# NazirNayal8/RbA

Hardware: AMD Instinct MI355X
Metric: images/sec @1024x2048 Swin-B-1dl (RbA inference hot path) (higher is better)
Workload: dtype f32 (f16x3 split-MFMA GEMMs, fp32 accumulate)

## Files before the change

### rba_amd/csrc/build.py

```python
import os
import subprocess
import sys
from concurrent.futures import ThreadPoolExecutor

HERE = os.path.dirname(os.path.abspath(__file__))
SOURCES = ["rba_reduce.hip", "rba_reduce_bwd.hip", "resample.hip", "ms_deform_attn.hip", "ms_deform_attn_bwd.hip", "masked_xattn.hip", "mask_logits.hip", "mask_logits_bwd.hip", "point_loss.hip", "outlier_tail.hip", "dense_hybrid_loss.hip", "pebal_loss.hip", "tta_merge.hip", "resize_u8.hip", "confusion.hip", "train_view.hip",
           "swin_window_attn.hip", "swin_attn_block.hip", "group_norm.hip", "layer_norm.hip", "skinny_linear.hip", "split_linear.hip", "split_linear_dma.hip", "split_linear_gnf.hip", "gaussian_blur.hip", "open_panoptic.hip", "dense_hybrid.hip", "patch_embed.hip", "token_linear.hip", "decoder_small.hip"]
HEADERS = ["common.h", "knobs.h", "bilinear_ac.h", "rba_reduce_kernels.h", "split_linear_dma.h", "split_linear_h3.h", "split_linear_h3q.h", "mlp_fused_h3.h", "swin_window_attn_h3.h", "swin_attn_block.h",
           os.path.join("..", "..", "include", "rba_hip.h")]
TUNE_SOURCES = [os.path.join("tune", "rba_reduce_tune.hip"), os.path.join("tune", "split_linear_tune.hip"), os.path.join("tune", "split_linear_ws.hip"), os.path.join("tune", "mlp_fused_h1.hip"), os.path.join("tune", "k5_timing.hip"), os.path.join("tune", "k5_wpe_ab.hip"), os.path.join("tune", "k5_wpe_plain.hip"), os.path.join("tune", "k5_persist.hip"), os.path.join("tune", "k7_timing.hip")] + [os.path.join("tune", f"gnf_form{f}_dbg{d}.hip") for f in (0, 1) for d in (0, 1)] + [os.path.join("tune", "gnf_form0_dbg1_unpacked.hip"), os.path.join("tune", "gnf_form1_dbg0_unpacked.hip")]
TUNE_LIB = os.path.join(HERE, "tune", "librba_tune.so")
LIB = os.path.join(HERE, "librba_hip.so")
KNOBS_LIB = os.path.join(HERE, "librba_hip_knobs.so")
KNOBS = ["-DRBA_TUNE_KNOBS"]
OBJ = os.path.join(HERE, "build")
HIPCC = os.environ.get("HIPCC", "/opt/rocm/bin/hipcc")
FLAGS = ["--offload-arch=gfx950", "-O3", "-std=c++17", "-fPIC", "-ffp-contract=fast", "-Wno-unused-result"]
NO_PACKED_FP32 = ["-Xclang", "-target-feature", "-Xclang", "-packed-fp32-ops"]
MFMA_SOURCES = ({"split_linear.hip", "split_linear_dma.hip", "mask_logits.hip", "mask_logits_bwd.hip", "masked_xattn.hip", "skinny_linear.hip"}
                if os.environ.get("RBA_NO_PACKED_FP32") == "1" else set())
UNPACKED_ALWAYS = {"split_linear_gnf.hip", "ms_deform_attn_bwd.hip", "point_loss.hip", "outlier_tail.hip", "dense_hybrid_loss.hip"}
UNPACKED_SOURCES = MFMA_SOURCES | UNPACKED_ALWAYS


def _run(cmd):
    r = subprocess.run(cmd, cwd=HERE, stderr=subprocess.PIPE, text=True)
    err = "\n".join(ln for ln in r.stderr.splitlines() if "not a recognized feature for this target" not in ln)
    if err.strip():
        print(err, file=sys.stderr, flush=True)
    if r.returncode:
        raise subprocess.CalledProcessError(r.returncode, cmd)


def _stale(target, deps) -> bool:
    if not os.path.exists(target):
        return True
    t = os.path.getmtime(target)
    return any(os.path.getmtime(d) > t for d in deps)


def stale() -> bool:
    return _stale(LIB, [os.path.join(HERE, f) for f in SOURCES + HEADERS])


def build(force: bool = False, verbose: bool = True, knobs: bool = False) -> str:
    lib = KNOBS_LIB if knobs else LIB
    if not force and not _stale(lib, [os.path.join(HERE, f) for f in SOURCES + HEADERS]):
        return lib
    obj_dir = os.path.join(OBJ, "knobs") if knobs else OBJ
    os.makedirs(obj_dir, exist_ok=True)
    hdrs = [os.path.join(HERE, h) for h in HEADERS]

    def compile_one(src):
        s, o = os.path.join(HERE, src), os.path.join(obj_dir, src.replace(".hip", ".o"))
        if force or _stale(o, [s] + hdrs):
            cmd = [HIPCC] + FLAGS + (KNOBS if knobs else []) + (NO_PACKED_FP32 if src in UNPACKED_SOURCES else []) + ["-c", s, "-o", o]
            if verbose:
                print(" ".join(cmd), flush=True)
            _run(cmd)
        return o

    with ThreadPoolExecutor(max_workers=min(8, os.cpu_count() or 1)) as ex:
        objs = list(ex.map(compile_one, SOURCES))
    _link_and_gate(objs, lib, verbose)
    return lib


def _link_and_gate(objs, lib, verbose):
    tmp = lib + ".unscanned"
    cmd = [HIPCC, "--offload-arch=gfx950", "-shared", "-fPIC"] + objs + ["-o", tmp]
    if verbose:
        print(" ".join(cmd), flush=True)
    subprocess.run(cmd, check=True, cwd=HERE)
    try:
        from . import isa_hazards
    except ImportError:
        sys.path.insert(0, HERE)
        import isa_hazards
    try:
        r = isa_hazards.gate(tmp)
    except Exception:
        os.remove(tmp)
        raise
    if verbose:
        print(f"isa_hazards: {os.path.basename(lib)}: {r['code_objects']} code objects clean (rules D, T, P)", flush=True)
    os.replace(tmp, lib)


def build_knobs(force: bool = False, verbose: bool = True) -> str:
    return build(force=force, verbose=verbose, knobs=True)


def build_tune(force: bool = False, verbose: bool = True) -> str:
    deps = [os.path.join(HERE, f) for f in TUNE_SOURCES + HEADERS + [os.path.join("tune", "split_linear_experiments.h"), os.path.join("tune", "rba_reduce_experiments.h")]]
    if not force and not _stale(TUNE_LIB, deps):
        return TUNE_LIB
    os.makedirs(OBJ, exist_ok=True)
    objs = []
    for src in TUNE_SOURCES:
        o = os.path.join(OBJ, "tune_" + os.path.basename(src).replace(".hip", ".o"))
        cmd = [HIPCC] + FLAGS + KNOBS + (NO_PACKED_FP32 if (MFMA_SOURCES and "split_linear" in src) or src.endswith("split_linear_ws.hip") or src.endswith("_unpacked.hip") or (src.endswith("mlp_fused_h1.hip") and os.environ.get("RBA_MLP1_UNPACKED") == "1") else []) + ["-c", os.path.join(HERE, src), "-o", o]
        if verbose:
            print(" ".join(cmd), flush=True)
        _run(cmd)
        objs.append(o)
    cmd = [HIPCC, "--offload-arch=gfx950", "-shared", "-fPIC"] + objs + ["-o", TUNE_LIB]
    if verbose:
        print(" ".join(cmd), flush=True)
    subprocess.run(cmd, check=True, cwd=HERE)
    return TUNE_LIB


if __name__ == "__main__":
    print(build(force="--force" in sys.argv))
    if "--knobs" in sys.argv:
        print(build_knobs(force="--force" in sys.argv))
    if "--tune" in sys.argv:
        print(build_tune(force="--force" in sys.argv))
```

### rba_amd/csrc/resample.hip

```cpp
#include "common.h"
#include "../../include/rba_hip.h"

namespace {

constexpr int CCHUNK = 4;

template <bool ADD, bool VEC4>
__global__ __launch_bounds__(256) void resample_kernel(const float* __restrict__ in, const float* __restrict__ add,
                                                       float* __restrict__ out, int C, int h, int w, int H, int W,
                                                       float sh, float sw, int wq) {
  const int xg = blockIdx.x * blockDim.x + threadIdx.x;
  const int y = blockIdx.y;
  if (xg >= wq) return;
  const int x0 = xg * 4;
  const BilinearTap ty = bilinear_tap(y, sh, h);
  BilinearTap tx[4];
#pragma unroll
  for (int r = 0; r < 4; ++r) tx[r] = bilinear_tap(x0 + r < W ? x0 + r : W - 1, sw, w);
  const int c0 = blockIdx.z * CCHUNK;
  auto one = [&](int c) {
    const float* r0 = in + ((int64_t)c * h + ty.i0) * w;
    const float* r1 = in + ((int64_t)c * h + ty.i1) * w;
    float v[4];
#pragma unroll
    for (int r = 0; r < 4; ++r) {
      const float top = tx[r].l0 * r0[tx[r].i0] + tx[r].l1 * r0[tx[r].i1];
      const float bot = tx[r].l0 * r1[tx[r].i0] + tx[r].l1 * r1[tx[r].i1];
      v[r] = ty.l0 * top + ty.l1 * bot;
    }
    const int64_t o = ((int64_t)c * H + y) * W + x0;
    if (VEC4) {
      f32x4 t = {v[0], v[1], v[2], v[3]};
      if (ADD) {
        t += *reinterpret_cast<const f32x4*>(add + o);
        *reinterpret_cast<f32x4*>(out + o) = t;
      } else {
        __builtin_nontemporal_store(t, reinterpret_cast<f32x4*>(out + o));
      }
    } else {
#pragma unroll
      for (int r = 0; r < 4; ++r)
        if (x0 + r < W) out[o + r] = ADD ? v[r] + add[o + r] : v[r];
    }
  };
  if (c0 + CCHUNK <= C) {
#pragma unroll
    for (int i = 0; i < CCHUNK; ++i) one(c0 + i);
  } else {
    for (int c = c0; c < C; ++c) one(c);
  }
}

struct GnFold {
  const float* mr;
  const float* gamma;
  const float* beta;
  int cpg;
  int relu;
};
__device__ __forceinline__ void gn_fold_coeff(const GnFold& g, int j, f32x4& a, f32x4& b) {
  const int grp = (j << 2) / g.cpg;
  const float mean = g.mr[2 * grp], rstd = g.mr[2 * grp + 1];
  const f32x4 ga = reinterpret_cast<const f32x4*>(g.gamma)[j], be = reinterpret_cast<const f32x4*>(g.beta)[j];
#pragma unroll
  for (int k = 0; k < 4; ++k) {
    a[k] = ga[k] * rstd;
    b[k] = be[k] - mean * a[k];
  }
}
__device__ __forceinline__ f32x4 gn_fold_apply(f32x4 v, const f32x4 a, const f32x4 b, int relu) {
#pragma unroll
  for (int k = 0; k < 4; ++k) {
    v[k] = fmaf(v[k], a[k], b[k]);
    v[k] = rba_clamp_below(v[k], rba_relu_floor(relu));
  }
  return v;
}

template <bool ADD, bool SOUT = false, bool GN = false>
__global__ __launch_bounds__(256) void resample_nhwc_kernel(const float* __restrict__ in, const float* __restrict__ add,
                                                            float* __restrict__ out, int C4, int h, int w, int H, int W, float sh,
                                                            float sw, int64_t row0 = 0, GnFold gin = GnFold{nullptr, nullptr, nullptr, 4, 0},
                                                            GnFold gadd = GnFold{nullptr, nullptr, nullptr, 4, 0}) {
  int64_t idx = (int64_t)blockIdx.x * 256 + threadIdx.x;
  int j;
  int64_t pix;
  if (SOUT) {
    const int64_t wv = idx >> 6;
    const int ln = (int)(idx & 63), nblk = C4 >> 3;
    j = (int)(wv % nblk) * 8 + (ln & 7);
    pix = (wv / nblk) * 8 + (ln >> 3);
    if (pix >= (int64_t)H * W) return;
    idx = pix * C4 + j;
  } else {
    const int64_t total = (int64_t)H * W * C4;
    if (idx >= total) return;
    j = (int)(idx % C4);
    pix = idx / C4;
  }
  const int x = (int)(pix % W), y = (int)(pix / W);
  const BilinearTap ty = bilinear_tap(y, sh, h), tx = bilinear_tap(x, sw, w);
  const f32x4* ip = reinterpret_cast<const f32x4*>(in) + j;
  f32x4 v00 = ip[((int64_t)ty.i0 * w + tx.i0) * C4], v01 = ip[((int64_t)ty.i0 * w + tx.i1) * C4];
  f32x4 v10 = ip[((int64_t)ty.i1 * w + tx.i0) * C4], v11 = ip[((int64_t)ty.i1 * w + tx.i1) * C4];
  if (GN && gin.mr) {
    f32x4 a, b;
    gn_fold_coeff(gin, j, a, b);
    v00 = gn_fold_apply(v00, a, b, gin.relu);
    v01 = gn_fold_apply(v01, a, b, gin.relu);
    v10 = gn_fold_apply(v10, a, b, gin.relu);
    v11 = gn_fold_apply(v11, a, b, gin.relu);
  }
  f32x4 r;
#pragma unroll
  for (int k = 0; k < 4; ++k) {
    const float top = tx.l0 * v00[k] + tx.l1 * v01[k];
    const float bot = tx.l0 * v10[k] + tx.l1 * v11[k];
    r[k] = ty.l0 * top + ty.l1 * bot;
  }
  if (ADD) {
    f32x4 av = reinterpret_cast<const f32x4*>(add)[idx];
    if (GN && gadd.mr) {
      f32x4 a, b;
      gn_fold_coeff(gadd, j, a, b);
      av = gn_fold_apply(av, a, b, gadd.relu);
    }
    r += av;
  }
  if (SOUT) {
    uint32_t hh[2], ll[2];
    rba_split_f16x2(r.x, r.y, hh[0], ll[0]);
    rba_split_f16x2(r.z, r.w, hh[1], ll[1]);
    const bool odd = j & 1;
    const uint32_t s0 = odd ? hh[0] : ll[0], s1 = odd ? hh[1] : ll[1];
    const uint32_t r0 = __builtin_amdgcn_mov_dpp(s0, 0xB1, 0xf, 0xf, true), r1 = __builtin_amdgcn_mov_dpp(s1, 0xB1, 0xf, 0xf, true);
    const rba_u32x4 piece = odd ? (rba_u32x4){r0, r1, ll[0], ll[1]} : (rba_u32x4){hh[0], hh[1], r0, r1};
    const int64_t row = row0 + pix;
    const int k8 = j >> 1;
    const int64_t off = ((row >> 5) * (int64_t)(C4 >> 3) + (k8 >> 2)) * 4096 + ((k8 & 1) * 2 + (odd ? 1 : 0)) * 1024 +
                        (((k8 >> 1) & 1) * 32 + (int)(row & 31)) * 16;
    *reinterpret_cast<rba_u32x4*>(reinterpret_cast<char*>(out) + off) = piece;
  } else {
    reinterpret_cast<f32x4*>(out)[idx] = r;
  }
}

}

extern "C" int rba_resample_bilinear_f32(const float* in, const float* add, float* out, int C, int h, int w, int H, int W,
                                         void* stream) {
  RBA_CHECK_ARG(C >= 0 && h >= 1 && w >= 1 && H >= 0 && W >= 0 && H <= 65535);
  if (C == 0 || H == 0 || W == 0) return 0;
  RBA_CHECK_ARG(in && out);
  const int cz = (C + CCHUNK - 1) / CCHUNK;
  RBA_CHECK_ARG(cz <= 65535);
  rba_begin();
  hipStream_t st = (hipStream_t)stream;
  const int wq = (W + 3) / 4;
  const int threads = wq >= 256 ? 256 : (wq >= 128 ? 128 : 64);
  dim3 grid((wq + threads - 1) / threads, H, cz);
  const float sh = (float)h / (float)H, sw = (float)w / (float)W;
  const bool vec4 = (W % 4 == 0) && ((((uintptr_t)out | (uintptr_t)add) & 15) == 0);
#define RBA_L(A, V) hipLaunchKernelGGL((resample_kernel<A, V>), grid, dim3(threads), 0, st, in, add, out, C, h, w, H, W, sh, sw, wq)
  if (add && vec4) RBA_L(true, true);
  else if (add) RBA_L(true, false);
  else if (vec4) RBA_L(false, true);
  else RBA_L(false, false);
#undef RBA_L
  return rba_launch_status();
}

extern "C" int rba_resample_bilinear_nhwc_f32(const float* in, const float* add, float* out, int C, int h, int w, int H, int W,
                                              void* stream) {
  RBA_CHECK_ARG(C >= 0 && (C & 3) == 0 && h >= 1 && w >= 1 && H >= 0 && W >= 0);
  if (C == 0 || H == 0 || W == 0) return 0;
  RBA_CHECK_ARG(in && out && ((((uintptr_t)in | (uintptr_t)out | (uintptr_t)add) & 15) == 0));
  const int64_t total = (int64_t)H * W * (C >> 2);
  RBA_CHECK_ARG((total + 255) / 256 <= 0x7fffffff);
  rba_begin();
  const float sh = (float)h / (float)H, sw = (float)w / (float)W;
  const dim3 grid((unsigned)((total + 255) / 256));
  if (add)
    hipLaunchKernelGGL(resample_nhwc_kernel<true>, grid, dim3(256), 0, (hipStream_t)stream, in, add, out, C >> 2, h, w, H, W, sh, sw);
  else
    hipLaunchKernelGGL(resample_nhwc_kernel<false>, grid, dim3(256), 0, (hipStream_t)stream, in, add, out, C >> 2, h, w, H, W, sh, sw);
  return rba_launch_status();
}

extern "C" int rba_resample_bilinear_nhwc_split_out_f32(const float* in, const float* add, void* out_frag, int C, int h, int w, int H, int W,
                                                        int64_t row0, void* stream) {
  RBA_CHECK_ARG(C >= 32 && (C % 32) == 0 && h >= 1 && w >= 1 && H >= 0 && W >= 0 && row0 >= 0);
  if (H == 0 || W == 0) return 0;
  RBA_CHECK_ARG(in && out_frag && (((uintptr_t)in | (uintptr_t)add | (uintptr_t)out_frag) & 15) == 0);
  const int64_t total = (((int64_t)H * W + 7) / 8) * 8 * (C >> 2);
  RBA_CHECK_ARG((total + 255) / 256 <= 0x7fffffffLL);
  rba_begin();
  const float sh = (float)h / (float)H, sw = (float)w / (float)W;
  const dim3 grid((unsigned)((total + 255) / 256));
  float* o = reinterpret_cast<float*>(out_frag);
  if (add)
    hipLaunchKernelGGL((resample_nhwc_kernel<true, true>), grid, dim3(256), 0, (hipStream_t)stream, in, add, o, C >> 2, h, w, H, W, sh, sw, row0);
  else
    hipLaunchKernelGGL((resample_nhwc_kernel<false, true>), grid, dim3(256), 0, (hipStream_t)stream, in, add, o, C >> 2, h, w, H, W, sh, sw, row0);
  return rba_launch_status();
}

extern "C" int rba_resample_bilinear_nhwc_gn_f32(const float* in, const float* in_mr, const float* in_gamma, const float* in_beta, int in_relu,
                                                 const float* add, const float* add_mr, const float* add_gamma, const float* add_beta, void* out,
                                                 int split_out, int C, int G, int h, int w, int H, int W, int64_t row0, void* stream) {
  RBA_CHECK_ARG(C >= 4 && (C % 4) == 0 && G >= 1 && (C % G) == 0 && ((C / G) % 4) == 0 && h >= 1 && w >= 1 && H >= 0 && W >= 0 && row0 >= 0);
  RBA_CHECK_ARG(!split_out || (C % 32) == 0);
  if (H == 0 || W == 0) return 0;
  RBA_CHECK_ARG(in && add && out && (!in_mr || (in_gamma && in_beta)) && (!add_mr || (add_gamma && add_beta)));
  RBA_CHECK_ARG((((uintptr_t)in | (uintptr_t)add | (uintptr_t)out | (uintptr_t)in_gamma | (uintptr_t)in_beta | (uintptr_t)add_gamma | (uintptr_t)add_beta) & 15) == 0);
  const int64_t total = split_out ? (((int64_t)H * W + 7) / 8) * 8 * (C >> 2) : (int64_t)H * W * (C >> 2);
  RBA_CHECK_ARG((total + 255) / 256 <= 0x7fffffffLL);
  rba_begin();
  const float sh = (float)h / (float)H, sw = (float)w / (float)W;
  const dim3 grid((unsigned)((total + 255) / 256));
  const GnFold gi{in_mr, in_gamma, in_beta, C / G, in_relu}, ga{add_mr, add_gamma, add_beta, C / G, 0};
  float* o = reinterpret_cast<float*>(out);
  if (split_out)
    hipLaunchKernelGGL((resample_nhwc_kernel<true, true, true>), grid, dim3(256), 0, (hipStream_t)stream, in, add, o, C >> 2, h, w, H, W, sh, sw, row0, gi, ga);
  else
    hipLaunchKernelGGL((resample_nhwc_kernel<true, false, true>), grid, dim3(256), 0, (hipStream_t)stream, in, add, o, C >> 2, h, w, H, W, sh, sw, row0, gi, ga);
  return rba_launch_status();
}
```

Before: 151.0.

## Compute multiple output rows per thread in GN-fused NHWC bilinear resample

Replaces the per-pixel GN-fused NHWC resample with a kernel where each thread handles R consecutive output rows (2 or 4) for one column and channel quad. For 2x upsampling with aligned taps, it loads R/2+1 source rows once and reuses the horizontally interpolated values across output rows, cutting redundant input loads and GN-fold arithmetic. The GN coefficient loads are hoisted and made branch-free, and a heuristic or knob picks R. A frozen copy of the old kernel is added to the tune library for comparison. The cost is more register pressure and a duplicated clamped-row path.

```diff
diff --git a/rba_amd/csrc/build.py b/rba_amd/csrc/build.py
--- a/rba_amd/csrc/build.py
+++ b/rba_amd/csrc/build.py
@@ -8,7 +8,7 @@
            "swin_window_attn.hip", "swin_attn_block.hip", "group_norm.hip", "layer_norm.hip", "skinny_linear.hip", "split_linear.hip", "split_linear_dma.hip", "split_linear_gnf.hip", "gaussian_blur.hip", "open_panoptic.hip", "dense_hybrid.hip", "patch_embed.hip", "token_linear.hip", "decoder_small.hip"]
 HEADERS = ["common.h", "knobs.h", "bilinear_ac.h", "rba_reduce_kernels.h", "split_linear_dma.h", "split_linear_h3.h", "split_linear_h3q.h", "mlp_fused_h3.h", "swin_window_attn_h3.h", "swin_attn_block.h",
            os.path.join("..", "..", "include", "rba_hip.h")]
-TUNE_SOURCES = [os.path.join("tune", "rba_reduce_tune.hip"), os.path.join("tune", "split_linear_tune.hip"), os.path.join("tune", "split_linear_ws.hip"), os.path.join("tune", "mlp_fused_h1.hip"), os.path.join("tune", "k5_timing.hip"), os.path.join("tune", "k5_wpe_ab.hip"), os.path.join("tune", "k5_wpe_plain.hip"), os.path.join("tune", "k5_persist.hip"), os.path.join("tune", "k7_timing.hip")] + [os.path.join("tune", f"gnf_form{f}_dbg{d}.hip") for f in (0, 1) for d in (0, 1)] + [os.path.join("tune", "gnf_form0_dbg1_unpacked.hip"), os.path.join("tune", "gnf_form1_dbg0_unpacked.hip")]
+TUNE_SOURCES = [os.path.join("tune", "rba_reduce_tune.hip"), os.path.join("tune", "split_linear_tune.hip"), os.path.join("tune", "split_linear_ws.hip"), os.path.join("tune", "mlp_fused_h1.hip"), os.path.join("tune", "k5_timing.hip"), os.path.join("tune", "k5_wpe_ab.hip"), os.path.join("tune", "k5_wpe_plain.hip"), os.path.join("tune", "k5_persist.hip"), os.path.join("tune", "k7_timing.hip"), os.path.join("tune", "fpn_path_frozen.hip")] + [os.path.join("tune", f"gnf_form{f}_dbg{d}.hip") for f in (0, 1) for d in (0, 1)] + [os.path.join("tune", "gnf_form0_dbg1_unpacked.hip"), os.path.join("tune", "gnf_form1_dbg0_unpacked.hip")]
 TUNE_LIB = os.path.join(HERE, "tune", "librba_tune.so")
 LIB = os.path.join(HERE, "librba_hip.so")
 KNOBS_LIB = os.path.join(HERE, "librba_hip_knobs.so")
diff --git a/rba_amd/csrc/resample.hip b/rba_amd/csrc/resample.hip
--- a/rba_amd/csrc/resample.hip
+++ b/rba_amd/csrc/resample.hip
@@ -1,5 +1,7 @@
 #include "common.h"
 #include "../../include/rba_hip.h"
+
+RBA_KNOB(rba_resample_rows, 0);
 
 namespace {
 
@@ -51,37 +53,24 @@
   }
 }
 
-struct GnFold {
-  const float* mr;
-  const float* gamma;
-  const float* beta;
-  int cpg;
-  int relu;
-};
-__device__ __forceinline__ void gn_fold_coeff(const GnFold& g, int j, f32x4& a, f32x4& b) {
-  const int grp = (j << 2) / g.cpg;
-  const float mean = g.mr[2 * grp], rstd = g.mr[2 * grp + 1];
-  const f32x4 ga = reinterpret_cast<const f32x4*>(g.gamma)[j], be = reinterpret_cast<const f32x4*>(g.beta)[j];
-#pragma unroll
-  for (int k = 0; k < 4; ++k) {
-    a[k] = ga[k] * rstd;
-    b[k] = be[k] - mean * a[k];
-  }
-}
-__device__ __forceinline__ f32x4 gn_fold_apply(f32x4 v, const f32x4 a, const f32x4 b, int relu) {
-#pragma unroll
-  for (int k = 0; k < 4; ++k) {
-    v[k] = fmaf(v[k], a[k], b[k]);
-    v[k] = rba_clamp_below(v[k], rba_relu_floor(relu));
-  }
-  return v;
-}
-
-template <bool ADD, bool SOUT = false, bool GN = false>
+__device__ __forceinline__ void resample_store_split(const f32x4 r, float* out, int64_t row, int j, int C4) {
+  uint32_t hh[2], ll[2];
+  rba_split_f16x2(r.x, r.y, hh[0], ll[0]);
+  rba_split_f16x2(r.z, r.w, hh[1], ll[1]);
+  const bool odd = j & 1;
+  const uint32_t s0 = odd ? hh[0] : ll[0], s1 = odd ? hh[1] : ll[1];
+  const uint32_t r0 = __builtin_amdgcn_mov_dpp(s0, 0xB1, 0xf, 0xf, true), r1 = __builtin_amdgcn_mov_dpp(s1, 0xB1, 0xf, 0xf, true);
+  const rba_u32x4 piece = odd ? (rba_u32x4){r0, r1, ll[0], ll[1]} : (rba_u32x4){hh[0], hh[1], r0, r1};
+  const int k8 = j >> 1;
+  const int64_t off = ((row >> 5) * (int64_t)(C4 >> 3) + (k8 >> 2)) * 4096 + ((k8 & 1) * 2 + (odd ? 1 : 0)) * 1024 +
+                      (((k8 >> 1) & 1) * 32 + (int)(row & 31)) * 16;
+  *reinterpret_cast<rba_u32x4*>(reinterpret_cast<char*>(out) + off) = piece;
+}
+
+template <bool ADD, bool SOUT = false>
 __global__ __launch_bounds__(256) void resample_nhwc_kernel(const float* __restrict__ in, const float* __restrict__ add,
                                                             float* __restrict__ out, int C4, int h, int w, int H, int W, float sh,
-                                                            float sw, int64_t row0 = 0, GnFold gin = GnFold{nullptr, nullptr, nullptr, 4, 0},
-                                                            GnFold gadd = GnFold{nullptr, nullptr, nullptr, 4, 0}) {
+                                                            float sw, int64_t row0 = 0) {
   int64_t idx = (int64_t)blockIdx.x * 256 + threadIdx.x;
   int j;
   int64_t pix;
@@ -103,14 +92,6 @@
   const f32x4* ip = reinterpret_cast<const f32x4*>(in) + j;
   f32x4 v00 = ip[((int64_t)ty.i0 * w + tx.i0) * C4], v01 = ip[((int64_t)ty.i0 * w + tx.i1) * C4];
   f32x4 v10 = ip[((int64_t)ty.i1 * w + tx.i0) * C4], v11 = ip[((int64_t)ty.i1 * w + tx.i1) * C4];
-  if (GN && gin.mr) {
-    f32x4 a, b;
-    gn_fold_coeff(gin, j, a, b);
-    v00 = gn_fold_apply(v00, a, b, gin.relu);
-    v01 = gn_fold_apply(v01, a, b, gin.relu);
-    v10 = gn_fold_apply(v10, a, b, gin.relu);
-    v11 = gn_fold_apply(v11, a, b, gin.relu);
-  }
   f32x4 r;
 #pragma unroll
   for (int k = 0; k < 4; ++k) {
@@ -118,31 +99,150 @@
     const float bot = tx.l0 * v10[k] + tx.l1 * v11[k];
     r[k] = ty.l0 * top + ty.l1 * bot;
   }
-  if (ADD) {
-    f32x4 av = reinterpret_cast<const f32x4*>(add)[idx];
-    if (GN && gadd.mr) {
-      f32x4 a, b;
-      gn_fold_coeff(gadd, j, a, b);
-      av = gn_fold_apply(av, a, b, gadd.relu);
-    }
-    r += av;
-  }
+  if (ADD) r += reinterpret_cast<const f32x4*>(add)[idx];
   if (SOUT) {
-    uint32_t hh[2], ll[2];
-    rba_split_f16x2(r.x, r.y, hh[0], ll[0]);
-    rba_split_f16x2(r.z, r.w, hh[1], ll[1]);
-    const bool odd = j & 1;
-    const uint32_t s0 = odd ? hh[0] : ll[0], s1 = odd ? hh[1] : ll[1];
-    const uint32_t r0 = __builtin_amdgcn_mov_dpp(s0, 0xB1, 0xf, 0xf, true), r1 = __builtin_amdgcn_mov_dpp(s1, 0xB1, 0xf, 0xf, true);
-    const rba_u32x4 piece = odd ? (rba_u32x4){r0, r1, ll[0], ll[1]} : (rba_u32x4){hh[0], hh[1], r0, r1};
-    const int64_t row = row0 + pix;
-    const int k8 = j >> 1;
-    const int64_t off = ((row >> 5) * (int64_t)(C4 >> 3) + (k8 >> 2)) * 4096 + ((k8 & 1) * 2 + (odd ? 1 : 0)) * 1024 +
-                        (((k8 >> 1) & 1) * 32 + (int)(row & 31)) * 16;
-    *reinterpret_cast<rba_u32x4*>(reinterpret_cast<char*>(out) + off) = piece;
+    resample_store_split(r, out, row0 + pix, j, C4);
   } else {
     reinterpret_cast<f32x4*>(out)[idx] = r;
   }
+}
+
+struct GnFold {
+  const float* mr;
+  const float* gamma;
+  const float* beta;
+  int cpg;
+  int relu;
+};
+struct GnRaw {
+  float mean, rstd;
+  f32x4 ga, be;
+};
+__device__ __forceinline__ GnRaw gn_fold_load(const GnFold& g, int j, const float* safe) {
+  const bool on = g.mr != nullptr;
+  const float* mr = on ? g.mr : safe;
+  const int grp = (j << 2) / g.cpg;
+  return GnRaw{mr[2 * grp], mr[2 * grp + 1], reinterpret_cast<const f32x4*>(on ? g.gamma : safe)[j], reinterpret_cast<const f32x4*>(on ? g.beta : safe)[j]};
+}
+__device__ __forceinline__ void gn_fold_coeff(const GnRaw& g, f32x4& a, f32x4& b) {
+#pragma unroll
+  for (int k = 0; k < 4; ++k) {
+    a[k] = g.ga[k] * g.rstd;
+    b[k] = fmaf(-g.mean, a[k], g.be[k]);
+  }
+}
+template <bool CLAMP>
+__device__ __forceinline__ f32x4 gn_fold_apply(f32x4 v, const f32x4 a, const f32x4 b, float floor = 0.f) {
+#pragma unroll
+  for (int k = 0; k < 4; ++k) {
+    v[k] = fmaf(v[k], a[k], b[k]);
+    if (CLAMP) v[k] = rba_clamp_below(v[k], floor);
+  }
+  return v;
+}
+
+__device__ __forceinline__ BilinearTap resample_tap(int dst, float scale, int in_size) {
+  float src = fmaf(scale, (float)dst + 0.5f, -0.5f);
+  src = src < 0.0f ? 0.0f : src;
+  int i0 = (int)src;
+  i0 = i0 < in_size - 1 ? i0 : in_size - 1;
+  BilinearTap t;
+  t.i0 = i0;
+  t.i1 = i0 < in_size - 1 ? i0 + 1 : i0;
+  t.l1 = src - (float)i0;
+  t.l0 = 1.0f - t.l1;
+  return t;
+}
+
+__device__ __forceinline__ f32x4 resample_lerp(float l0, const f32x4 a, float l1, const f32x4 b) {
+  return (f32x4){fmaf(l1, b.x, l0 * a.x), fmaf(l0, a.y, l1 * b.y), fmaf(l1, b.z, l0 * a.z), fmaf(l0, a.w, l1 * b.w)};
+}
+
+template <bool SOUT, int R>
+__global__ __launch_bounds__(256) void resample_nhwc_gn_kernel(const float* __restrict__ in, const float* __restrict__ add, float* __restrict__ out, int C4, int h,
+                                                               int w, int H, int W, float sh, float sw, int64_t row0, GnFold gin, GnFold gadd) {
+  constexpr int NS = R / 2 + 1;
+  int x, j;
+  if (SOUT) {
+    const unsigned wv = blockIdx.x * 4 + (threadIdx.x >> 6), nblk = (unsigned)C4 >> 3, xg = wv / nblk;
+    const int ln = threadIdx.x & 63;
+    j = (int)(wv - xg * nblk) * 8 + (ln & 7);
+    x = (int)xg * 8 + (ln >> 3);
+    if (x >= W) return;
+  } else {
+    const unsigned e = blockIdx.x * 256 + threadIdx.x;
+    if (e >= (unsigned)W * (unsigned)C4) return;
+    x = (int)(e / (unsigned)C4);
+    j = (int)(e - (unsigned)x * (unsigned)C4);
+  }
+  const int ya = R * (int)blockIdx.y - 1;
+  const BilinearTap tx = resample_tap(x, sw, w);
+  const f32x4* ip = reinterpret_cast<const f32x4*>(in) + j;
+  const f32x4* ap = reinterpret_cast<const f32x4*>(add) + j;
+  int pix[R];
+  BilinearTap ty[R];
+  f32x4 av[R];
+#pragma unroll
+  for (int r = 0; r < R; ++r) {
+    const int y = ya + r < 0 ? 0 : (ya + r < H ? ya + r : H - 1);
+    pix[r] = y * W + x;
+    ty[r] = resample_tap(y, sh, h);
+    av[r] = ap[(int64_t)pix[r] * C4];
+  }
+  const bool fold_in = gin.mr != nullptr, fold_add = gadd.mr != nullptr;
+  const GnRaw raw_in = gn_fold_load(gin, j, in), raw_add = gn_fold_load(gadd, j, add);
+  const float floor_in = rba_relu_floor(gin.relu);
+  f32x4 ai, bi, aa, ba;
+  auto hrow = [&](f32x4 v0, f32x4 v1) {
+    if (fold_in) {
+      v0 = gn_fold_apply<true>(v0, ai, bi, floor_in);
+      v1 = gn_fold_apply<true>(v1, ai, bi, floor_in);
+    }
+    return resample_lerp(tx.l0, v0, tx.l1, v1);
+  };
+  auto emit = [&](int r, const f32x4 top, const f32x4 bot) {
+    f32x4 v = resample_lerp(ty[r].l0, top, ty[r].l1, bot);
+    v += fold_add ? gn_fold_apply<false>(av[r], aa, ba) : av[r];
+    if (ya + r < 0 || ya + r >= H) return;
+    if (SOUT) resample_store_split(v, out, row0 + pix[r], j, C4);
+    else reinterpret_cast<f32x4*>(out)[(int64_t)pix[r] * C4 + j] = v;
+  };
+  const int s0 = ty[0].i0;
+  bool aligned = true;
+#pragma unroll
+  for (int r = 0; r < R; ++r) aligned = aligned && ty[r].i0 == s0 + (r >> 1) && ty[r].i1 == s0 + (r >> 1) + 1;
+  if (aligned) {
+    f32x4 t0[NS], t1[NS];
+#pragma unroll
+    for (int k = 0; k < NS; ++k) {
+      t0[k] = ip[(int64_t)((s0 + k) * w + tx.i0) * C4];
+      t1[k] = ip[(int64_t)((s0 + k) * w + tx.i1) * C4];
+    }
+    gn_fold_coeff(raw_in, ai, bi);
+    gn_fold_coeff(raw_add, aa, ba);
+    f32x4 hs[NS];
+#pragma unroll
+    for (int k = 0; k < NS; ++k) hs[k] = hrow(t0[k], t1[k]);
+#pragma unroll
+    for (int r = 0; r < R; ++r) emit(r, hs[r >> 1], hs[(r >> 1) + 1]);
+  } else {
+    gn_fold_coeff(raw_in, ai, bi);
+    gn_fold_coeff(raw_add, aa, ba);
+#pragma unroll
+    for (int r = 0; r < R; ++r) {
+      const int o0 = ty[r].i0 * w, o1 = ty[r].i1 * w;
+      const f32x4 v00 = ip[(int64_t)(o0 + tx.i0) * C4], v01 = ip[(int64_t)(o0 + tx.i1) * C4];
+      const f32x4 v10 = ip[(int64_t)(o1 + tx.i0) * C4], v11 = ip[(int64_t)(o1 + tx.i1) * C4];
+      emit(r, hrow(v00, v01), hrow(v10, v11));
+    }
+  }
+}
+
+template <bool SOUT, int R>
+bool resample_gn_grid(int C4, int H, int W, dim3& grid) {
+  const int64_t gx = SOUT ? ((int64_t)((W + 7) / 8) * (C4 >> 3) + 3) / 4 : ((int64_t)W * C4 + 255) / 256, gy = ((int64_t)H + R) / R;
+  grid = dim3((unsigned)gx, (unsigned)gy);
+  return gx <= 0x3fffffff && gy <= 65535;
 }
 
 }
@@ -213,16 +313,29 @@
   if (H == 0 || W == 0) return 0;
   RBA_CHECK_ARG(in && add && out && (!in_mr || (in_gamma && in_beta)) && (!add_mr || (add_gamma && add_beta)));
   RBA_CHECK_ARG((((uintptr_t)in | (uintptr_t)add | (uintptr_t)out | (uintptr_t)in_gamma | (uintptr_t)in_beta | (uintptr_t)add_gamma | (uintptr_t)add_beta) & 15) == 0);
-  const int64_t total = split_out ? (((int64_t)H * W + 7) / 8) * 8 * (C >> 2) : (int64_t)H * W * (C >> 2);
-  RBA_CHECK_ARG((total + 255) / 256 <= 0x7fffffffLL);
-  rba_begin();
+  const int C4 = C >> 2;
+  RBA_CHECK_ARG((int64_t)H * W < (int64_t)1 << 31 && (int64_t)h * w < (int64_t)1 << 31 && (int64_t)W * C4 < (int64_t)1 << 31);
   const float sh = (float)h / (float)H, sw = (float)w / (float)W;
-  const dim3 grid((unsigned)((total + 255) / 256));
   const GnFold gi{in_mr, in_gamma, in_beta, C / G, in_relu}, ga{add_mr, add_gamma, add_beta, C / G, 0};
   float* o = reinterpret_cast<float*>(out);
-  if (split_out)
-    hipLaunchKernelGGL((resample_nhwc_kernel<true, true, true>), grid, dim3(256), 0, (hipStream_t)stream, in, add, o, C >> 2, h, w, H, W, sh, sw, row0, gi, ga);
-  else
-    hipLaunchKernelGGL((resample_nhwc_kernel<true, false, true>), grid, dim3(256), 0, (hipStream_t)stream, in, add, o, C >> 2, h, w, H, W, sh, sw, row0, gi, ga);
+  hipStream_t st = (hipStream_t)stream;
+  dim3 grid;
+#define RBA_L(S, R)                                                                                                                                  \
+  do {                                                                                                                                               \
+    RBA_CHECK_ARG((resample_gn_grid<S, R>(C4, H, W, grid)));                                                                                         \
+    rba_begin();                                                                                                                                     \
+    hipLaunchKernelGGL((resample_nhwc_gn_kernel<S, R>), grid, dim3(256), 0, st, in, add, o, C4, h, w, H, W, sh, sw, row0, gi, ga);                   \
+  } while (0)
+  dim3 g4;
+  const bool fits4 = split_out ? resample_gn_grid<true, 4>(C4, H, W, g4) : resample_gn_grid<false, 4>(C4, H, W, g4);
+  const bool four = rba_resample_rows == 4 || (rba_resample_rows == 0 && fits4 && (int64_t)g4.x * g4.y >= 2048);
+  if (split_out) {
+    if (four) RBA_L(true, 4);
+    else RBA_L(true, 2);
+  } else {
+    if (four) RBA_L(false, 4);
+    else RBA_L(false, 2);
+  }
+#undef RBA_L
   return rba_launch_status();
 }
diff --git a/rba_amd/csrc/tune/fpn_path_frozen.hip b/rba_amd/csrc/tune/fpn_path_frozen.hip
--- /dev/null
+++ b/rba_amd/csrc/tune/fpn_path_frozen.hip
@@ -0,0 +1,121 @@
+#include "../common.h"
+
+namespace {
+
+struct FrozenGnFold {
+  const float* mr;
+  const float* gamma;
+  const float* beta;
+  int cpg;
+  int relu;
+};
+__device__ __forceinline__ void frozen_gn_fold_coeff(const FrozenGnFold& g, int j, f32x4& a, f32x4& b) {
+  const int grp = (j << 2) / g.cpg;
+  const float mean = g.mr[2 * grp], rstd = g.mr[2 * grp + 1];
+  const f32x4 ga = reinterpret_cast<const f32x4*>(g.gamma)[j], be = reinterpret_cast<const f32x4*>(g.beta)[j];
+#pragma unroll
+  for (int k = 0; k < 4; ++k) {
+    a[k] = ga[k] * rstd;
+    b[k] = be[k] - mean * a[k];
+  }
+}
+__device__ __forceinline__ f32x4 frozen_gn_fold_apply(f32x4 v, const f32x4 a, const f32x4 b, int relu) {
+#pragma unroll
+  for (int k = 0; k < 4; ++k) {
+    v[k] = fmaf(v[k], a[k], b[k]);
+    v[k] = rba_clamp_below(v[k], rba_relu_floor(relu));
+  }
+  return v;
+}
+
+template <bool ADD, bool SOUT = false, bool GN = false>
+__global__ __launch_bounds__(256) void frozen_resample_nhwc_kernel(const float* __restrict__ in, const float* __restrict__ add,
+                                                                   float* __restrict__ out, int C4, int h, int w, int H, int W, float sh,
+                                                                   float sw, int64_t row0 = 0, FrozenGnFold gin = FrozenGnFold{nullptr, nullptr, nullptr, 4, 0},
+                                                                   FrozenGnFold gadd = FrozenGnFold{nullptr, nullptr, nullptr, 4, 0}) {
+  int64_t idx = (int64_t)blockIdx.x * 256 + threadIdx.x;
+  int j;
+  int64_t pix;
+  if (SOUT) {
+    const int64_t wv = idx >> 6;
+    const int ln = (int)(idx & 63), nblk = C4 >> 3;
+    j = (int)(wv % nblk) * 8 + (ln & 7);
+    pix = (wv / nblk) * 8 + (ln >> 3);
+    if (pix >= (int64_t)H * W) return;
+    idx = pix * C4 + j;
+  } else {
+    const int64_t total = (int64_t)H * W * C4;
+    if (idx >= total) return;
+    j = (int)(idx % C4);
+    pix = idx / C4;
+  }
+  const int x = (int)(pix % W), y = (int)(pix / W);
+  const BilinearTap ty = bilinear_tap(y, sh, h), tx = bilinear_tap(x, sw, w);
+  const f32x4* ip = reinterpret_cast<const f32x4*>(in) + j;
+  f32x4 v00 = ip[((int64_t)ty.i0 * w + tx.i0) * C4], v01 = ip[((int64_t)ty.i0 * w + tx.i1) * C4];
+  f32x4 v10 = ip[((int64_t)ty.i1 * w + tx.i0) * C4], v11 = ip[((int64_t)ty.i1 * w + tx.i1) * C4];
+  if (GN && gin.mr) {
+    f32x4 a, b;
+    frozen_gn_fold_coeff(gin, j, a, b);
+    v00 = frozen_gn_fold_apply(v00, a, b, gin.relu);
+    v01 = frozen_gn_fold_apply(v01, a, b, gin.relu);
+    v10 = frozen_gn_fold_apply(v10, a, b, gin.relu);
+    v11 = frozen_gn_fold_apply(v11, a, b, gin.relu);
+  }
+  f32x4 r;
+#pragma unroll
+  for (int k = 0; k < 4; ++k) {
+    const float top = tx.l0 * v00[k] + tx.l1 * v01[k];
+    const float bot = tx.l0 * v10[k] + tx.l1 * v11[k];
+    r[k] = ty.l0 * top + ty.l1 * bot;
+  }
+  if (ADD) {
+    f32x4 av = reinterpret_cast<const f32x4*>(add)[idx];
+    if (GN && gadd.mr) {
+      f32x4 a, b;
+      frozen_gn_fold_coeff(gadd, j, a, b);
+      av = frozen_gn_fold_apply(av, a, b, gadd.relu);
+    }
+    r += av;
+  }
+  if (SOUT) {
+    uint32_t hh[2], ll[2];
+    rba_split_f16x2(r.x, r.y, hh[0], ll[0]);
+    rba_split_f16x2(r.z, r.w, hh[1], ll[1]);
+    const bool odd = j & 1;
+    const uint32_t s0 = odd ? hh[0] : ll[0], s1 = odd ? hh[1] : ll[1];
+    const uint32_t r0 = __builtin_amdgcn_mov_dpp(s0, 0xB1, 0xf, 0xf, true), r1 = __builtin_amdgcn_mov_dpp(s1, 0xB1, 0xf, 0xf, true);
+    const rba_u32x4 piece = odd ? (rba_u32x4){r0, r1, ll[0], ll[1]} : (rba_u32x4){hh[0], hh[1], r0, r1};
+    const int64_t row = row0 + pix;
+    const int k8 = j >> 1;
+    const int64_t off = ((row >> 5) * (int64_t)(C4 >> 3) + (k8 >> 2)) * 4096 + ((k8 & 1) * 2 + (odd ? 1 : 0)) * 1024 +
+                        (((k8 >> 1) & 1) * 32 + (int)(row & 31)) * 16;
+    *reinterpret_cast<rba_u32x4*>(reinterpret_cast<char*>(out) + off) = piece;
+  } else {
+    reinterpret_cast<f32x4*>(out)[idx] = r;
+  }
+}
+
+}
+
+extern "C" int rba_tune_resample_bilinear_nhwc_gn_frozen_f32(const float* in, const float* in_mr, const float* in_gamma, const float* in_beta, int in_relu,
+                                                             const float* add, const float* add_mr, const float* add_gamma, const float* add_beta, void* out,
+                                                             int split_out, int C, int G, int h, int w, int H, int W, int64_t row0, void* stream) {
+  RBA_CHECK_ARG(C >= 4 && (C % 4) == 0 && G >= 1 && (C % G) == 0 && ((C / G) % 4) == 0 && h >= 1 && w >= 1 && H >= 0 && W >= 0 && row0 >= 0);
+  RBA_CHECK_ARG(!split_out || (C % 32) == 0);
+  if (H == 0 || W == 0) return 0;
+  RBA_CHECK_ARG(in && add && out && (!in_mr || (in_gamma && in_beta)) && (!add_mr || (add_gamma && add_beta)));
+  RBA_CHECK_ARG((((uintptr_t)in | (uintptr_t)add | (uintptr_t)out | (uintptr_t)in_gamma | (uintptr_t)in_beta | (uintptr_t)add_gamma | (uintptr_t)add_beta) & 15) == 0);
+  const int64_t total = split_out ? (((int64_t)H * W + 7) / 8) * 8 * (C >> 2) : (int64_t)H * W * (C >> 2);
+  RBA_CHECK_ARG((total + 255) / 256 <= 0x7fffffffLL);
+  rba_begin();
+  const float sh = (float)h / (float)H, sw = (float)w / (float)W;
+  const dim3 grid((unsigned)((total + 255) / 256));
+  const FrozenGnFold gi{in_mr, in_gamma, in_beta, C / G, in_relu}, ga{add_mr, add_gamma, add_beta, C / G, 0};
+  float* o = reinterpret_cast<float*>(out);
+  if (split_out)
+    hipLaunchKernelGGL((frozen_resample_nhwc_kernel<true, true, true>), grid, dim3(256), 0, (hipStream_t)stream, in, add, o, C >> 2, h, w, H, W, sh, sw, row0, gi, ga);
+  else
+    hipLaunchKernelGGL((frozen_resample_nhwc_kernel<true, false, true>), grid, dim3(256), 0, (hipStream_t)stream, in, add, o, C >> 2, h, w, H, W, sh, sw, row0, gi, ga);
+  return rba_launch_status();
+}
```

Result: no change. 151.9, median of 6 (+0.6%).
